# AHupuJR/REFID

Measured on AMD Instinct MI355X. Metric: interpolated frames/sec (train step) GoPro 256x256 11+1, higher is better.
Workload: dtype f32

## Files before the change

refid_amd/csrc/wgrad_wino24.hip:

```cpp
#include "common.h"
#include "wgrad_args.h"
#include <cstdlib>
#include <cstring>
#include <type_traits>
#include <vector>

#ifndef REFID_W24_ABLATE
#define REFID_W24_ABLATE 0
#endif
#define W24_NO_DMA (REFID_W24_ABLATE == 1 || REFID_W24_ABLATE == 5 || REFID_W24_ABLATE == 6)
#define W24_NO_MFMA (REFID_W24_ABLATE == 2)
#define W24_NO_LDS (REFID_W24_ABLATE == 3 || REFID_W24_ABLATE == 6)
#define W24_NO_BAR (REFID_W24_ABLATE == 4 || REFID_W24_ABLATE == 5 || REFID_W24_ABLATE == 6)

namespace {

__device__ __forceinline__ float w24_fake(float seed) { asm volatile("" : "+v"(seed)); return seed; }

constexpr int IT = 32;
constexpr int TC = 4;
constexpr int GH = 4, GW = 4 * TC;
constexpr int XH = GH + 2, XW = GW + 2;
constexpr int X_BYTES = XH * XW * IT * 4;
constexpr int GS_BYTES = GH * GW * 32 * 4;
constexpr int buf_bytes(int ns) { return X_BYTES + ns * GS_BYTES; }
constexpr int lds24_bytes(int ns) { return 2 * buf_bytes(ns); }
constexpr int NXI = 24;
typedef __attribute__((address_space(3))) void* lds_ptr24;
typedef __attribute__((address_space(3))) const float lds_cf24;
typedef float f32x2 __attribute__((ext_vector_type(2)));

template <int AH, int BH>
__device__ __forceinline__ f32x2 w24_pair(f32x2 a, f32x2 b) {
    f32x2 d;
    if constexpr (AH == 0 && BH == 0) asm("v_pk_mov_b32 %0, %1, %2 op_sel:[0,0]" : "=v"(d) : "v"(a), "v"(b));
    else if constexpr (AH == 1 && BH == 0) asm("v_pk_mov_b32 %0, %1, %2 op_sel:[1,0]" : "=v"(d) : "v"(a), "v"(b));
    else if constexpr (AH == 0 && BH == 1) asm("v_pk_mov_b32 %0, %1, %2 op_sel:[0,1]" : "=v"(d) : "v"(a), "v"(b));
    else asm("v_pk_mov_b32 %0, %1, %2 op_sel:[1,1]" : "=v"(d) : "v"(a), "v"(b));
    return d;
}

struct W24Args {
    const float* g[REFID_WGRAD_MAX_GROUPS]; const float* inA[REFID_WGRAD_MAX_GROUPS]; const float* inB[REFID_WGRAD_MAX_GROUPS];
    int groups;
    int ldG, Co;
    int ldA, ldB, Ca, Ctot;
    float* slabs; float* bslabs;
    int N, H, W, Ho, Wo, pad;
    int tilesX, tilesY, ntiles, nsplit;
    int CoP, CiP;
    int accum;
    int Hin, Win, ncoT;
};

template <int I>
struct W24Row {
    static constexpr int XR = XW * IT, GR = GW * 32, GSUB = GH * GW * 32;
    static constexpr int XA = I == 0 ? 0 : (I == 2 ? 2 : (I == 3 ? 3 : 1));
    static constexpr int XB = I == 0 ? 2 : (I == 2 ? 1 : (I == 3 ? 1 : 2));
    static constexpr bool XPLUS = I == 1;

    template <class T>
    static __device__ __forceinline__ T x_comb(T a, T b) { return XPLUS ? a + b : a - b; }
    static __device__ __forceinline__ void x_rows(lds_cf24* const (&xb)[4], int s, f32x2 (&t)[6]) {
#pragma unroll
        for (int c = 0; c < 4; ++c) {
            const int col = 4 * s + 2 + c;
            lds_cf24* p = xb[col & 3] + (col & ~3) * IT;
            const f32x2 a = W24_NO_LDS ? f32x2{w24_fake(1.f + c), w24_fake(2.f)} : f32x2{p[XA * XR], p[XA * XR + 4 * IT]};
            const f32x2 b = W24_NO_LDS ? f32x2{w24_fake(3.f + c), w24_fake(4.f)} : f32x2{p[XB * XR], p[XB * XR + 4 * IT]};
            t[2 + c] = x_comb(a, b);
        }
    }
    static __device__ __forceinline__ f32x2 x_rows01(lds_cf24* xe) {
        if (W24_NO_LDS) return f32x2{w24_fake(5.f), w24_fake(6.f)};
        return x_comb(f32x2{xe[XA * XR], xe[XA * XR + IT]}, f32x2{xe[XB * XR], xe[XB * XR + IT]});
    }
    static __device__ __forceinline__ void g_rows(lds_cf24* const (&gb)[4], int s, int sub, f32x2 (&x)[4]) {
#pragma unroll
        for (int c = 0; c < 4; ++c) {
            const int col = 4 * s + c;
            lds_cf24* p = gb[col & 3] + sub * GSUB + (col & ~3) * 32;
            if (W24_NO_LDS) { x[c] = f32x2{w24_fake(7.f + c), w24_fake(8.f + sub)}; continue; }
            if constexpr (I == 0) x[c] = f32x2{p[0], p[4 * 32]};
            else if constexpr (I == 3) x[c] = f32x2{p[GR], p[GR + 4 * 32]};
            else {
                const f32x2 g0 = f32x2{p[0], p[4 * 32]}, g1 = f32x2{p[GR], p[GR + 4 * 32]};
                x[c] = I == 1 ? g0 + g1 : g0 - g1;
            }
        }
    }
    static __device__ __forceinline__ void v_cols(const f32x2 (&t)[6], f32x2 (&v)[6]) {
        v[0] = 4.f * t[0] + (-5.f * t[2] + t[4]);
        v[1] = (t[3] + t[4]) - 4.f * (t[1] + t[2]);
        v[2] = 4.f * (t[1] - t[2]) + (t[4] - t[3]);
        const f32x2 d42 = t[4] - t[2], d31 = t[3] - t[1];
        v[3] = 2.f * d31 + d42;
        v[4] = d42 - 2.f * d31;
        v[5] = 4.f * t[1] + (-5.f * t[3] + t[5]);
    }
    static __device__ __forceinline__ void z_cols(const f32x2 (&x)[4], f32x2 (&z)[6]) {
        const f32x2 e = x[0] + x[2], o = x[1] + x[3], e4 = 4.f * x[2] + x[0], o4 = 4.f * x[3] + x[1];
        z[0] = x[0]; z[1] = e + o; z[2] = e - o; z[3] = 2.f * o4 + e4; z[4] = e4 - 2.f * o4; z[5] = x[3];
    }
};

template <int NS, bool DOWN>
__global__ __launch_bounds__(256, NS == 2 ? 2 : 3) void wgrad_wino24_kernel(const W24Args a) {
    constexpr int OT = 32 * NS, BUF_BYTES = buf_bytes(NS), XPS = DOWN ? 2 : 1;
    extern __shared__ __attribute__((aligned(16))) char smem[];
    const int tid = threadIdx.x, lane = tid & 63;
    const int wave = __builtin_amdgcn_readfirstlane(tid >> 6);
    const int li = lane & 31, kh = lane >> 5;
    const int phase = DOWN ? blockIdx.z / a.ncoT : 0, php = phase >> 1, phq = phase & 1;
    const int co0 = (DOWN ? blockIdx.z % a.ncoT : blockIdx.z) * OT, ci0 = blockIdx.y * IT;
    const int split = blockIdx.x;
    const int Hin = DOWN ? a.Hin : a.H, Win = DOWN ? a.Win : a.W;

    const bool xFromA = ci0 < a.Ca || ci0 >= a.Ctot;
    const int xld = xFromA ? a.ldA : a.ldB;
    const long long gpixAll = (long long)a.N * a.Ho * a.Wo, xpixAll = (long long)a.N * Hin * Win;
    const int limG = (int)min(gpixAll * a.ldG * 4, 0x7fffffffLL), limX = (int)min(xpixAll * xld * 4, 0x7fffffffLL);
    const int ntAll = a.ntiles * a.groups;
    const int chunk = (ntAll + a.nsplit - 1) / a.nsplit;
    const int p0 = min(split * chunk, ntAll), p1 = min(p0 + chunk, ntAll);

    int qg, qn, qy, qx;
    {
        int t = p0 < ntAll ? p0 : 0;
        qg = t / a.ntiles; t -= qg * a.ntiles;
        qx = t % a.tilesX; t /= a.tilesX;
        qy = t % a.tilesY; qn = t / a.tilesY;
    }
    const int xq = ci0 + (lane & 7) * 4, xt = ci0 + (lane & 31), gq = co0 + (lane & 7) * 4;
    const int xlc = ((lane >> 3) * XPS * xld + (xFromA ? xq : xq - a.Ca)) * 4;
    const int xlt = ((lane >> 5) * XPS * xld + (xFromA ? xt : xt - a.Ca)) * 4;
    const int glc = ((lane >> 3) * a.ldG + gq) * 4;
    const bool fullch = ci0 + IT <= a.Ctot && co0 + OT <= a.Co;
    constexpr int OOB = 0x7ff00000;
    const int xRowB = XPS * Win * xld * 4, gRowB = a.Wo * a.ldG * 4;
    auto x_origin = [&](int n, int ty, int tx) {
        return ((n * Hin + XPS * (ty * GH - a.pad) + php) * Win + XPS * (tx * GW - a.pad) + phq) * xld * 4;
    };
    const float* gPtr = a.g[qg];
    const float* xPtr = xFromA ? a.inA[qg] : a.inB[qg];
    int xTile = x_origin(qn, qy, qx);
    int gTile = ((qn * a.Ho + qy * GH) * a.Wo + qx * GW) * a.ldG * 4;
    auto request = [&](int buf) {
        const int oy0 = qy * GH, ox0 = qx * GW;
        const int iy0 = oy0 - a.pad, ix0 = ox0 - a.pad;
        const __amdgpu_buffer_rsrc_t rsG = __builtin_amdgcn_make_buffer_rsrc(const_cast<float*>(gPtr), 0, limG, 0x00020000);
        const __amdgpu_buffer_rsrc_t rsX = __builtin_amdgcn_make_buffer_rsrc(const_cast<float*>(xPtr), 0, limX, 0x00020000);
        char* xdst = smem + buf * BUF_BYTES;
        char* gdst = xdst + X_BYTES;
        const bool fast = fullch && ix0 >= 0 && ix0 + XW <= a.W && ox0 + GW <= a.Wo && xld * 8 * XPS * 4 < 0x100000 && a.ldG * 8 * 4 < 0x100000;
        const int q0 = NS == 2 ? (wave < 2 ? wave : 3 * wave - 4) : 2 * (wave - 2), nq = NS == 2 ? (wave < 2 ? 1 : 3) : (wave < 2 ? 0 : 2);
        if (fast) {
#pragma unroll
            for (int k = 0; k < 2; ++k) {
                const int r = wave + 4 * k;
                if (r < XH && !W24_NO_DMA) {
                    const int base = (unsigned)(iy0 + r) < (unsigned)a.H ? xTile + r * xRowB : OOB;
                    char* dst = xdst + r * (XW * IT * 4);
                    __builtin_amdgcn_raw_ptr_buffer_load_lds(rsX, (lds_ptr24)dst, 16, base + xlc, 0, 0, 0);
                    __builtin_amdgcn_raw_ptr_buffer_load_lds(rsX, (lds_ptr24)(dst + 1024), 16, base + 8 * XPS * xld * 4 + xlc, 0, 0, 0);
                    __builtin_amdgcn_raw_ptr_buffer_load_lds(rsX, (lds_ptr24)(dst + 2048), 4, base + 16 * XPS * xld * 4 + xlt, 0, 0, 0);
                }
            }
#pragma unroll
            for (int k = 0; k < 3; ++k) {
                if (k < nq && !W24_NO_DMA) {
                    const int q = q0 + k, r = q & 3, sub = q >> 2;
                    const int base = oy0 + r < a.Ho ? gTile + r * gRowB + sub * 128 : OOB;
                    char* dst = gdst + sub * GS_BYTES + r * (GW * 32 * 4);
                    __builtin_amdgcn_raw_ptr_buffer_load_lds(rsG, (lds_ptr24)dst, 16, base + glc, 0, 0, 0);
                    __builtin_amdgcn_raw_ptr_buffer_load_lds(rsG, (lds_ptr24)(dst + 1024), 16, base + 8 * a.ldG * 4 + glc, 0, 0, 0);
                }
            }
        } else {
            const int l8 = lane >> 3, l32 = lane >> 5;
            const int xbadq = xq < a.Ctot ? 0 : -1, xbadt = xt < a.Ctot ? 0 : -1;
            const int gbad0 = gq < a.Co ? 0 : -1, gbad1 = gq + 32 < a.Co ? 0 : -1;
            const int cx0 = (unsigned)(ix0 + l8) < (unsigned)a.W ? 0 : -1;
            const int cx1 = (unsigned)(ix0 + 8 + l8) < (unsigned)a.W ? 0 : -1;
            const int cxt = (unsigned)(ix0 + 16 + l32) < (unsigned)a.W ? 0 : -1;
            const int cg0 = ox0 + l8 < a.Wo ? 0 : -1, cg1 = ox0 + 8 + l8 < a.Wo ? 0 : -1;
#pragma unroll
            for (int k = 0; k < 2; ++k) {
                const int r = wave + 4 * k;
                if (r < XH && !W24_NO_DMA) {
                    const int rbad = (unsigned)(iy0 + r) < (unsigned)a.H ? 0 : -1;
                    const int base = xTile + r * xRowB;
                    char* dst = xdst + r * (XW * IT * 4);
                    __builtin_amdgcn_raw_ptr_buffer_load_lds(rsX, (lds_ptr24)dst, 16, (base + xlc) | xbadq | rbad | cx0, 0, 0, 0);
                    __builtin_amdgcn_raw_ptr_buffer_load_lds(rsX, (lds_ptr24)(dst + 1024), 16,
                                                             (base + 8 * XPS * xld * 4 + xlc) | xbadq | rbad | cx1, 0, 0, 0);
                    __builtin_amdgcn_raw_ptr_buffer_load_lds(rsX, (lds_ptr24)(dst + 2048), 4,
                                                             (base + 16 * XPS * xld * 4 + xlt) | xbadt | rbad | cxt, 0, 0, 0);
                }
            }
#pragma unroll
            for (int k = 0; k < 3; ++k) {
                if (k < nq && !W24_NO_DMA) {
                    const int q = q0 + k, r = q & 3, sub = q >> 2;
                    const int rbad = oy0 + r < a.Ho ? 0 : -1;
                    const int base = gTile + r * gRowB + sub * 128;
                    const int gbad = sub ? gbad1 : gbad0;
                    char* dst = gdst + sub * GS_BYTES + r * (GW * 32 * 4);
                    __builtin_amdgcn_raw_ptr_buffer_load_lds(rsG, (lds_ptr24)dst, 16, (base + glc) | gbad | rbad | cg0, 0, 0, 0);
                    __builtin_amdgcn_raw_ptr_buffer_load_lds(rsG, (lds_ptr24)(dst + 1024), 16,
                                                             (base + 8 * a.ldG * 4 + glc) | gbad | rbad | cg1, 0, 0, 0);
                }
            }
        }
        if (REFID_W24_ABLATE == 7) return;
        qx += 1;
        if (qx != a.tilesX) {
            xTile += GW * XPS * xld * 4;
            gTile += GW * a.ldG * 4;
        } else {
            qx = 0;
            qy += 1;
            if (qy == a.tilesY) {
                qy = 0;
                qn += 1;
                if (qn == a.N) {
                    qn = 0;
                    qg = min(qg + 1, a.groups - 1);
                    gPtr = a.g[qg];
                    xPtr = xFromA ? a.inA[qg] : a.inB[qg];
                }
            }
            xTile = x_origin(qn, qy, 0);
            gTile = (qn * a.Ho + qy * GH) * a.Wo * a.ldG * 4;
        }
    };

    f32x16 acc[6][NS];
#pragma unroll
    for (int j = 0; j < 6; ++j)
#pragma unroll
        for (int sm = 0; sm < NS; ++sm)
#pragma unroll
            for (int r = 0; r < 16; ++r) acc[j][sm][r] = 0.f;
    float bs[NS];
#pragma unroll
    for (int sm = 0; sm < NS; ++sm) bs[sm] = 0.f;

    static_assert(BUF_BYTES % 256 == 0 && (BUF_BYTES + X_BYTES + (NS - 1) * GS_BYTES + 4 * GW * 32 * 4) / 256 < 256, "ds_read2st64 offset range");
    lds_cf24* xe = (lds_cf24*)smem + (2 * kh) * (XW * IT) + li;
    lds_cf24* ge = (lds_cf24*)(smem + X_BYTES) + (2 * kh) * (GW * 32) + li;
    lds_cf24* xb[4] = {xe, xe + IT, xe + 2 * IT, xe + 3 * IT};
    lds_cf24* gb[4] = {ge, ge + 32, ge + 2 * 32, ge + 3 * 32};
    asm volatile("" : "+v"(xb[0]), "+v"(xb[1]), "+v"(xb[2]), "+v"(xb[3]), "+v"(xe));
    asm volatile("" : "+v"(gb[0]), "+v"(gb[1]), "+v"(gb[2]), "+v"(gb[3]));

    auto kloop = [&](auto TI) {
        constexpr int I = decltype(TI)::value;
        using R = W24Row<I>;
        auto tile = [&](auto BUF) {
            constexpr int BO = decltype(BUF)::value * (BUF_BYTES / 4);
            lds_cf24* xbb[4] = {xb[0] + BO, xb[1] + BO, xb[2] + BO, xb[3] + BO};
            lds_cf24* gbb[4] = {gb[0] + BO, gb[1] + BO, gb[2] + BO, gb[3] + BO};
            f32x2 t[6], p4, p5;
#pragma unroll
            for (int s = 0; s < TC; s += 2) {
                R::x_rows(xbb, s, t);
                if (s == 0) {
                    const f32x2 a01 = R::x_rows01(xe + BO);
                    t[0] = w24_pair<0, 0>(a01, t[4]);
                    t[1] = w24_pair<1, 0>(a01, t[5]);
                } else {
                    t[0] = w24_pair<1, 0>(p4, t[4]);
                    t[1] = w24_pair<1, 0>(p5, t[5]);
                }
                p4 = t[4]; p5 = t[5];
                f32x2 v[6];
                R::v_cols(t, v);
#pragma unroll
                for (int sm = 0; sm < NS; ++sm) {
                    f32x2 x[4], z[6];
                    R::g_rows(gbb, s, sm, x);
                    R::z_cols(x, z);
                    if constexpr (I == 1) bs[sm] += z[1][0] + z[1][1];
#pragma unroll
                    for (int h = 0; h < 2; ++h)
#pragma unroll
                        for (int j = 0; j < 6; ++j) {
                            if (W24_NO_MFMA) { asm volatile("" :: "v"(v[j][h]), "v"(z[j][h])); continue; }
                            acc[j][sm] = __builtin_amdgcn_mfma_f32_32x32x2f32(v[j][h], z[j][h], acc[j][sm], 0, 0, 0);
                        }
                }
            }
        };
        auto sync = [&] {
            __builtin_amdgcn_s_waitcnt(0x0F70);
            if (!W24_NO_BAR) __builtin_amdgcn_s_barrier();
            __builtin_amdgcn_sched_barrier(0);
        };
        const int npairs = (p1 - p0) >> 1;
        if (p0 < p1) request(0);
        for (int i = 0; i < npairs; ++i) {
            sync();
            request(1);
            tile(std::integral_constant<int, 0>{});
            sync();
            if (p0 + 2 * i + 2 < p1) request(0);
            tile(std::integral_constant<int, 1>{});
        }
        if ((p1 - p0) & 1) {
            sync();
            tile(std::integral_constant<int, 0>{});
        }
    };
    switch (wave) {
        case 0: kloop(std::integral_constant<int, 0>{}); break;
        case 1: kloop(std::integral_constant<int, 1>{}); break;
        case 2: kloop(std::integral_constant<int, 2>{}); break;
        default: kloop(std::integral_constant<int, 3>{}); break;
    }

#pragma unroll
    for (int j = 0; j < 6; ++j) {
        float* sl = a.slabs + ((long long)((split * (DOWN ? 4 : 1) + phase) * NXI + wave * 6 + j) * a.CoP) * a.CiP;
#pragma unroll
        for (int sm = 0; sm < NS; ++sm) {
            const int co = co0 + sm * 32 + li;
#pragma unroll
            for (int qd = 0; qd < 4; ++qd) {
                const int ci = ci0 + 8 * qd + 4 * kh;
                f32x4 vv;
#pragma unroll
                for (int k = 0; k < 4; ++k) vv[k] = acc[j][sm][4 * qd + k];
                f32x4* dst = reinterpret_cast<f32x4*>(sl + (long long)co * a.CiP + ci);
                if (a.accum) vv += *dst;
                *dst = vv;
            }
        }
    }
    if (a.bslabs != nullptr && blockIdx.y == 0 && phase == 0 && wave == 1) {
#pragma unroll
        for (int sm = 0; sm < NS; ++sm) {
            const float tot = bs[sm] + __shfl_xor(bs[sm], 32, 64);
            if (kh == 0) {
                float* dst = a.bslabs + (long long)split * a.CoP + co0 + sm * 32 + li;
                *dst = a.accum ? *dst + tot : tot;
            }
        }
    }
}

struct W24rArgs {
    const float* slabs; const float* bslabs; float* dw; float* db;
    int nsplit, Co, Ci, CoP, CiP, iBase, iTotal, perGroup;
    int nsplitW;
    int down;
};

__device__ __forceinline__ void w24_fold_body(const float* __restrict__ slabs, float* __restrict__ part, long long slabFloats,
                                              int nsplit, int S, int piece, int s) {
    const long long off = ((long long)piece * 256 + threadIdx.x) * 4;
    if (off >= slabFloats) return;
    const f32x4* p = reinterpret_cast<const f32x4*>(slabs + off);
    const long long st4 = slabFloats / 4;
    f32x4 a0 = {0.f, 0.f, 0.f, 0.f}, a1 = a0;
    int k = s;
    for (; k + S < nsplit; k += 2 * S) { a0 += p[k * st4]; a1 += p[(k + S) * st4]; }
    if (k < nsplit) a0 += p[k * st4];
    *reinterpret_cast<f32x4*>(part + (long long)s * slabFloats + off) = a0 + a1;
}
__global__ __launch_bounds__(256) void wgrad_wino24_fold_kernel(const float* __restrict__ slabs, float* __restrict__ part,
                                                                long long slabFloats, int nsplit, int S) {
    w24_fold_body(slabs, part, slabFloats, nsplit, S, blockIdx.x, blockIdx.y);
}

constexpr int FOLD_BATCH = 96;
struct FoldJob { const float* slabs; float* part; long long slabFloats; int nsplit, S; };
struct FoldBatch { FoldJob job[FOLD_BATCH]; int blk0[FOLD_BATCH + 1]; int n; };
static_assert(sizeof(FoldBatch) <= 4096, "kernel-argument block");
__global__ __launch_bounds__(256) void wgrad_fold_batch_kernel(const FoldBatch b) {
    int j = 0;
    for (int k = 1; k < b.n; ++k) j = (int)blockIdx.x >= b.blk0[k] ? k : j;
    const FoldJob& f = b.job[j];
    const int blk = (int)blockIdx.x - b.blk0[j];
    const int pieces = (int)((f.slabFloats / 4 + 255) / 256);
    w24_fold_body(f.slabs, f.part, f.slabFloats, f.nsplit, f.S, blk % pieces, blk / pieces);
}
thread_local std::vector<FoldJob> fold_queue;

__device__ __forceinline__ void w24_reduce_body(const W24rArgs& a, const int blk, float* part) {
    const long long plane = (long long)a.CoP * a.CiP;
    const long long slabStride = NXI * plane;
    const int lpe = a.perGroup, eb = 256 / lpe;
    const int el = threadIdx.x % eb, sub = threadIdx.x / eb;
    const long long e = (long long)blk * eb + el;
    const bool live = e < (long long)a.Co * a.Ci;
    const int ci = live ? (int)(e % a.Ci) : 0, co = live ? (int)(e / a.Ci) : 0;
    {
        const float* p = a.slabs + (long long)co * a.CiP + ci;
        float u[NXI];
#pragma unroll
        for (int x = 0; x < NXI; ++x) u[x] = 0.f;
        if (live) {
            for (int k = sub; k < a.nsplitW; k += lpe) {
#pragma unroll
                for (int x = 0; x < NXI; ++x) u[x] += p[k * slabStride + x * plane];
            }
        }
        if (lpe > 1) {
#pragma unroll
            for (int x = 0; x < NXI; ++x) part[threadIdx.x * (NXI + 1) + x] = u[x];
            __syncthreads();
            if (sub == 0) {
                for (int s2 = 1; s2 < lpe; ++s2) {
#pragma unroll
                    for (int x = 0; x < NXI; ++x) u[x] += part[(s2 * eb + el) * (NXI + 1) + x];
                }
            }
        }
        if (live && sub == 0) {
            constexpr float c4 = 0.25f, c6 = 1.f / 6.f, c12 = 1.f / 12.f, c24 = 1.f / 24.f;
            float dg[9];
#pragma unroll
            for (int pp = 0; pp < 3; ++pp) {
                float t[6];
#pragma unroll
                for (int j = 0; j < 6; ++j) {
                    const float m = 0.5f * (u[6 + j] + u[12 + j]), d = 0.5f * (u[6 + j] - u[12 + j]);
                    t[j] = pp == 0 ? u[j] + m : (pp == 1 ? d : m + u[18 + j]);
                }
                const float s12 = t[1] + t[2], d21 = t[2] - t[1], s34 = t[3] + t[4], d34 = t[3] - t[4];
                dg[pp * 3 + 0] = c4 * t[0] - c6 * s12 + c24 * s34;
                dg[pp * 3 + 1] = c6 * d21 + c12 * d34;
                dg[pp * 3 + 2] = c6 * (s34 - s12) + t[5];
            }
            float* dst = a.dw + ((long long)co * a.iTotal + a.iBase + ci) * 9;
#pragma unroll
            for (int k = 0; k < 9; ++k) dst[k] += dg[k];
        }
    }
    if (a.db != nullptr && blk == 0) {
        for (int c2 = threadIdx.x; c2 < a.Co; c2 += 256) {
            float s = 0.f;
            for (int k = 0; k < a.nsplit; ++k) s += a.bslabs[(long long)k * a.CoP + c2];
            a.db[c2] += s;
        }
    }
}

__global__ __launch_bounds__(256) void wgrad_wino24_reduce_kernel(const W24rArgs a) {
    __shared__ float part[256 * (NXI + 1)];
    w24_reduce_body(a, blockIdx.x, part);
}

__device__ __forceinline__ void w24_reduce_down_body(const W24rArgs& a, const int blk) {
    const long long plane = (long long)a.CoP * a.CiP;
    const long long slabStride = 4 * NXI * plane;
    const long long gid = (long long)blk * 256 + threadIdx.x;
    const long long e = gid >> 2;
    const int ph = (int)(gid & 3);
    const bool live = e < (long long)a.Co * a.Ci;
    const int ci = live ? (int)(e % a.Ci) : 0, co = live ? (int)(e / a.Ci) : 0;
    if (live) {
        const float* p = a.slabs + (long long)co * a.CiP + ci + ph * NXI * plane;
        float u[NXI];
#pragma unroll
        for (int x = 0; x < NXI; ++x) u[x] = 0.f;
        for (int k = 0; k < a.nsplitW; ++k) {
#pragma unroll
            for (int x = 0; x < NXI; ++x) u[x] += p[k * slabStride + x * plane];
        }
        constexpr float c4 = 0.25f, c6 = 1.f / 6.f, c12 = 1.f / 12.f, c24 = 1.f / 24.f;
        float* dst = a.dw + ((long long)co * a.iTotal + a.iBase + ci) * 16;
#pragma unroll
        for (int pp = 0; pp < 3; ++pp) {
            const int ky = 2 * pp + (ph >> 1) - 1;
            float t[6];
#pragma unroll
            for (int j = 0; j < 6; ++j) {
                const float m = 0.5f * (u[6 + j] + u[12 + j]), d = 0.5f * (u[6 + j] - u[12 + j]);
                t[j] = pp == 0 ? u[j] + m : (pp == 1 ? d : m + u[18 + j]);
            }
            const float s12 = t[1] + t[2], d21 = t[2] - t[1], s34 = t[3] + t[4], d34 = t[3] - t[4];
            const float r3[3] = {c4 * t[0] - c6 * s12 + c24 * s34, c6 * d21 + c12 * d34, c6 * (s34 - s12) + t[5]};
            if (ky < 0 || ky > 3) continue;
#pragma unroll
            for (int q = 0; q < 3; ++q) {
                const int kx = 2 * q + (ph & 1) - 1;
                if (kx >= 0 && kx <= 3) dst[ky * 4 + kx] += r3[q];
            }
        }
    }
    if (a.db != nullptr && blk == 0) {
        for (int c2 = threadIdx.x; c2 < a.Co; c2 += 256) {
            float sacc = 0.f;
            for (int k = 0; k < a.nsplit; ++k) sacc += a.bslabs[(long long)k * a.CoP + c2];
            a.db[c2] += sacc;
        }
    }
}

__global__ __launch_bounds__(256) void wgrad_wino24_reduce_down_kernel(const W24rArgs a) { w24_reduce_down_body(a, blockIdx.x); }

struct W24rBatch { W24rArgs job[REFID_FINISH_BATCH]; int blk0[REFID_FINISH_BATCH + 1]; int n; };
static_assert(sizeof(W24rBatch) <= 4096, "kernel-argument block");
__global__ __launch_bounds__(256) void wgrad_wino24_reduce_batch_kernel(const W24rBatch b) {
    __shared__ float part[256 * (NXI + 1)];
    int j = 0;
    for (int k = 1; k < b.n; ++k) j = (int)blockIdx.x >= b.blk0[k] ? k : j;
    const int blk = (int)blockIdx.x - b.blk0[j];
    if (b.job[j].down) w24_reduce_down_body(b.job[j], blk);
    else w24_reduce_body(b.job[j], blk, part);
}

struct W24rQueued { W24rArgs r; int nblocks; };
thread_local std::vector<W24rQueued> w24_queue;

struct Geo24 { int ncoT, nciT, tilesX, tilesY, ntiles, nsplit, CoP, CiP; };

int ns_of(const refid_wgrad_desc* d) { return d->c_o <= 32 ? 1 : 2; }
bool is_down(const refid_wgrad_desc* d) { return d->kh == 4; }

Geo24 geo24_of(const refid_wgrad_desc* d) {
    Geo24 g;
    const int OT = 32 * ns_of(d);
    g.ncoT = cdiv(d->c_o, OT);
    const int ci_geo = (d->phase != 0) ? d->i_total - d->i_base : d->c_a + d->c_b;
    g.nciT = cdiv(ci_geo > d->c_a + d->c_b ? ci_geo : d->c_a + d->c_b, IT);
    g.tilesX = cdiv(d->wo, GW);
    g.tilesY = cdiv(d->ho, GH);
    g.ntiles = g.tilesX * g.tilesY * d->n;
    static const int wgs = []() { const char* e = getenv("REFID_W24_WGS"); return e ? atoi(e) : 512; }();
    int want = cdiv(ns_of(d) == 1 ? wgs * 3 / 2 : wgs, g.ncoT * g.nciT * (is_down(d) ? 4 : 1));
    if (want >= 8) want = want / 8 * 8;
    if (want < 1) want = 1;
    if (want > g.ntiles) want = g.ntiles;
    g.nsplit = want;
    g.CoP = g.ncoT * OT;
    g.CiP = g.nciT * IT;
    return g;
}

}

int refid_slab_fold_count(long long slabFloats, int nsplit) {
    if (nsplit < 2) return 0;
    const long long pieces = (slabFloats / 4 + 255) / 256;
    int S = (int)((2048 + pieces - 1) / pieces);
    if (S > 16) S = 16;
    if (S >= nsplit) S = nsplit / 2;
    return S < 1 ? 1 : S;
}
int refid_launch_slab_fold(const float* slabs, float* part, long long slabFloats, int nsplit, int S, hipStream_t st) {
    static const bool batch_folds = !(getenv("REFID_FOLD_BATCH") && getenv("REFID_FOLD_BATCH")[0] == '0');
    if (batch_folds && refid_finish_defer_now()) {
        fold_queue.push_back({slabs, part, slabFloats, nsplit, S});
        return 0;
    }
    hipLaunchKernelGGL(wgrad_wino24_fold_kernel, dim3((unsigned)((slabFloats / 4 + 255) / 256), S), dim3(256), 0, st, slabs, part,
                       slabFloats, nsplit, S);
    REFID_LAUNCH_CHECK("wgrad_slab_fold");
    return 0;
}

int refid_slab_fold_flush(hipStream_t st) {
    size_t at = 0;
    while (at < fold_queue.size()) {
        FoldBatch b;
        memset(&b, 0, sizeof(b));
        int n = 0;
        long long blk = 0;
        for (; n < FOLD_BATCH && at < fold_queue.size(); ++n, ++at) {
            const FoldJob& f = fold_queue[at];
            const long long nb = ((f.slabFloats / 4 + 255) / 256) * f.S;
            if (n > 0 && blk + nb > 0x3fffffffLL) break;
            b.job[n] = f;
            b.blk0[n] = (int)blk;
            blk += nb;
        }
        b.blk0[n] = (int)blk; b.n = n;
        hipLaunchKernelGGL(wgrad_fold_batch_kernel, dim3((unsigned)blk), dim3(256), 0, st, b);
        if (hipGetLastError() != hipSuccess) { fold_queue.clear(); refid_set_error("wgrad_fold_batch: launch failed"); return 1; }
    }
    fold_queue.clear();
    return 0;
}

int refid_wino24_finish_flush(hipStream_t st) {
    size_t at = 0;
    while (at < w24_queue.size()) {
        W24rBatch b;
        memset(&b, 0, sizeof(b));
        int n = 0, blk = 0;
        for (; n < REFID_FINISH_BATCH && at < w24_queue.size(); ++n, ++at) {
            b.job[n] = w24_queue[at].r;
            b.blk0[n] = blk;
            blk += w24_queue[at].nblocks;
        }
        b.blk0[n] = blk; b.n = n;
        hipLaunchKernelGGL(wgrad_wino24_reduce_batch_kernel, dim3(blk), dim3(256), 0, st, b);
        if (hipGetLastError() != hipSuccess) { w24_queue.clear(); refid_set_error("wgrad_wino24_reduce_batch: launch failed"); return 1; }
    }
    w24_queue.clear();
    return 0;
}

namespace {
long long slab_floats(const refid_wgrad_desc* d, const Geo24& g) { return (long long)(is_down(d) ? 4 : 1) * NXI * g.CoP * g.CiP; }
}

size_t refid_wgrad_wino24_workspace_bytes(const refid_wgrad_desc* d) {
    const Geo24 g = geo24_of(d);
    const long long slab = slab_floats(d, g);
    return ((size_t)g.nsplit * slab + (size_t)g.nsplit * g.CoP + (size_t)refid_slab_fold_count(slab, g.nsplit) * slab) * sizeof(float);
}

int refid_wgrad_wino24_launch(const refid_wgrad_desc* d, hipStream_t st) {
    static std::atomic<unsigned long long> attr_done{0}, attr_done1{0}, attr_done2{0}, attr_done3{0};
    if (int rc = refid_lds_attr_once(attr_done, &wgrad_wino24_kernel<2, false>, lds24_bytes(2), "wgrad_wino24")) return rc;
    if (int rc = refid_lds_attr_once(attr_done1, &wgrad_wino24_kernel<1, false>, lds24_bytes(1), "wgrad_wino24<1>")) return rc;
    if (int rc = refid_lds_attr_once(attr_done2, &wgrad_wino24_kernel<2, true>, lds24_bytes(2), "wgrad_wino24<down>")) return rc;
    if (int rc = refid_lds_attr_once(attr_done3, &wgrad_wino24_kernel<1, true>, lds24_bytes(1), "wgrad_wino24<1, down>")) return rc;
    const Geo24 g = geo24_of(d);
    const bool down = is_down(d);
    const long long slab = slab_floats(d, g);
    if (down)
        REFID_CHECK(d->kw == 4 && d->stride == 2 && d->pad == 1 && d->h % 2 == 0 && d->w % 2 == 0 && d->ho == d->h / 2 && d->wo == d->w / 2,
                    "wgrad (algo 7): a 4x4 stride-2 pad-1 conv over an even-sized input");
    REFID_CHECK(d->c_b == 0 || d->c_a % IT == 0, "wgrad (Winograd 2x4 tiles): c_a must be a multiple of %d for two sources", IT);
    REFID_CHECK(d->ld_g % 4 == 0 && d->ld_a % 4 == 0 && (d->c_b == 0 || d->ld_b % 4 == 0) && d->c_o % 4 == 0 &&
                    d->c_a % 4 == 0 && d->c_b % 4 == 0,
                "wgrad (Winograd 2x4 tiles): pitches and channel counts must be multiples of 4 floats (16-byte LDS-DMA pieces)");
    {
        const long long lim = 0x7fffffffLL;
        REFID_CHECK((long long)d->n * d->ho * d->wo * d->ld_g * 4 < lim && (long long)d->n * d->h * d->w * d->ld_a * 4 < lim &&
                        (d->c_b == 0 || (long long)d->n * d->h * d->w * d->ld_b * 4 < lim),
                    "wgrad (Winograd 2x4 tiles): tensor too large for 32-bit buffer offsets (use algo 0)");
    }
    W24Args a;
    const int ngrp = d->groups > 1 ? d->groups : 1;
    REFID_CHECK(ngrp <= REFID_WGRAD_MAX_GROUPS, "wgrad: at most %d grouped time steps", REFID_WGRAD_MAX_GROUPS);
    for (int k = 0; k < REFID_WGRAD_MAX_GROUPS; ++k) {
        const bool on = k > 0 && k < ngrp;
        a.g[k] = k == 0 ? d->g : (on ? d->g_more[k - 1] : d->g);
        a.inA[k] = k == 0 ? d->in_a : (on ? d->in_a_more[k - 1] : d->in_a);
        a.inB[k] = k == 0 ? d->in_b : (on ? d->in_b_more[k - 1] : d->in_b);
        REFID_CHECK(a.g[k] && a.inA[k] && (d->c_b == 0 || a.inB[k]), "wgrad: null tensor pointer in group %d", k);
        REFID_CHECK(((uintptr_t)a.g[k] | (uintptr_t)a.inA[k] | (uintptr_t)(d->c_b ? a.inB[k] : nullptr)) % 16 == 0,
                    "wgrad (Winograd 2x4 tiles): tensors must be 16-byte aligned (group %d)", k);
    }
    a.groups = ngrp;
    a.ldG = d->ld_g; a.Co = d->c_o;
    a.ldA = d->ld_a; a.ldB = d->ld_b;
    a.Ca = d->c_a; a.Ctot = d->c_a + d->c_b;
    a.slabs = d->slabs;
    a.bslabs = d->db ? d->slabs + (size_t)g.nsplit * slab : nullptr;
    a.N = d->n; a.H = d->h; a.W = d->w; a.Ho = d->ho; a.Wo = d->wo; a.pad = d->pad;
    a.Hin = d->h; a.Win = d->w; a.ncoT = g.ncoT;
    if (down) { a.H = d->ho; a.W = d->wo; a.pad = 1; }
    a.tilesX = g.tilesX; a.tilesY = g.tilesY; a.ntiles = g.ntiles; a.nsplit = g.nsplit;
    a.CoP = g.CoP; a.CiP = g.CiP;
    a.accum = (d->phase == 2);
    if (d->phase != 3) {
        if (down) {
            if (ns_of(d) == 1)
                hipLaunchKernelGGL((wgrad_wino24_kernel<1, true>), dim3(g.nsplit, g.nciT, 4 * g.ncoT), dim3(256), lds24_bytes(1), st, a);
            else
                hipLaunchKernelGGL((wgrad_wino24_kernel<2, true>), dim3(g.nsplit, g.nciT, 4 * g.ncoT), dim3(256), lds24_bytes(2), st, a);
        } else if (ns_of(d) == 1)
            hipLaunchKernelGGL((wgrad_wino24_kernel<1, false>), dim3(g.nsplit, g.nciT, g.ncoT), dim3(256), lds24_bytes(1), st, a);
        else
            hipLaunchKernelGGL((wgrad_wino24_kernel<2, false>), dim3(g.nsplit, g.nciT, g.ncoT), dim3(256), lds24_bytes(2), st, a);
        REFID_LAUNCH_CHECK("wgrad_wino24");
    }
    if (d->phase == 1 || d->phase == 2) return 0;
    W24rArgs r;
    r.slabs = a.slabs; r.bslabs = a.bslabs; r.dw = d->dw; r.db = d->db;
    r.nsplit = g.nsplit; r.Co = d->o_real;
    int nred = g.nsplit;
    if (const int S = refid_slab_fold_count(slab, g.nsplit)) {
        const long long slabFloats = slab;
        float* part = d->slabs + (size_t)g.nsplit * slab + (size_t)g.nsplit * g.CoP;
        if (int rc = refid_launch_slab_fold(a.slabs, part, slabFloats, g.nsplit, S, st)) return rc;
        r.slabs = part;
        nred = S;
    }
    r.Ci = (d->phase == 0 && a.Ctot < d->i_total - d->i_base) ? a.Ctot : d->i_total - d->i_base;
    r.CoP = g.CoP; r.CiP = g.CiP; r.iBase = d->i_base; r.iTotal = d->i_total;
    const long long total = (long long)r.Co * r.Ci;
    int lpe = 1;
    while (lpe < 16 && (long long)lpe * 2 * total <= 65536 && lpe * 2 <= nred) lpe *= 2;
    r.perGroup = lpe;
    r.nsplitW = nred;
    r.down = down ? 1 : 0;
    if (refid_finish_defer_now()) {
        for (const W24rQueued& q : w24_queue)
            if (q.r.dw == r.dw && q.r.iBase == r.iBase) {
                if (int rc = refid_slab_fold_flush(st)) return rc;
                if (int rc = refid_wino24_finish_flush(st)) return rc;
                break;
            }
        w24_queue.push_back({r, down ? (int)((total * 4 + 255) / 256) : (int)((total + 256 / lpe - 1) / (256 / lpe))});
        return 0;
    }
    if (down) {
        hipLaunchKernelGGL(wgrad_wino24_reduce_down_kernel, dim3((int)((total * 4 + 255) / 256)), dim3(256), 0, st, r);
        REFID_LAUNCH_CHECK("wgrad_wino24_reduce_down");
        return 0;
    }
    hipLaunchKernelGGL(wgrad_wino24_reduce_kernel, dim3((int)((total + 256 / lpe - 1) / (256 / lpe))), dim3(256), 0, st, r);
    REFID_LAUNCH_CHECK("wgrad_wino24_reduce");
    return 0;
}
```

Measured before the change: 525.6.

## Add eight-wave Winograd wgrad variant sharing gradient tiles across two input-channel blocks

Adds an X8 form of the Winograd 2x4 weight-gradient kernel with 512 threads. Two groups of four waves each handle a 32-channel input block and share one staged gradient tile in LDS. The new form uses a triple-buffered LDS pipeline with partial waitcnt so two tile loads can be in flight. It is meant to halve gradient tile traffic per input channel and to hide load latency better. In exchange it runs at one workgroup per CU with a larger LDS footprint. It is selected by default for non-down 64-output-channel layers with at least 256x256 output pixels and more than 32 input channels.

Measured after the change: 529.5 (median of 6 runs). Within noise of the previous version (+0.7%).

```diff
diff --git a/refid_amd/csrc/wgrad_wino24.hip b/refid_amd/csrc/wgrad_wino24.hip
--- a/refid_amd/csrc/wgrad_wino24.hip
+++ b/refid_amd/csrc/wgrad_wino24.hip
@@ -16,6 +16,11 @@
 namespace {
 
 __device__ __forceinline__ float w24_fake(float seed) { asm volatile("" : "+v"(seed)); return seed; }
+__device__ __forceinline__ int w24_lane_now() {
+    int l;
+    asm volatile("v_mbcnt_lo_u32_b32 %0, -1, 0\n\tv_mbcnt_hi_u32_b32 %0, -1, %0" : "=v"(l));
+    return l;
+}
 
 constexpr int IT = 32;
 constexpr int TC = 4;
@@ -25,6 +30,9 @@
 constexpr int GS_BYTES = GH * GW * 32 * 4;
 constexpr int buf_bytes(int ns) { return X_BYTES + ns * GS_BYTES; }
 constexpr int lds24_bytes(int ns) { return 2 * buf_bytes(ns); }
+constexpr int X8_XOFF(int h, int b) { return (3 * h + b) * X_BYTES; }
+constexpr int X8_GOFF(int b) { return 6 * X_BYTES + b * 2 * GS_BYTES; }
+constexpr int LDS24X8_BYTES = X8_GOFF(3);
 constexpr int NXI = 24;
 typedef __attribute__((address_space(3))) void* lds_ptr24;
 typedef __attribute__((address_space(3))) const float lds_cf24;
@@ -105,15 +113,17 @@
     }
 };
 
-template <int NS, bool DOWN>
-__global__ __launch_bounds__(256, NS == 2 ? 2 : 3) void wgrad_wino24_kernel(const W24Args a) {
+template <int NS, bool DOWN, bool X8 = false>
+__global__ __launch_bounds__(X8 ? 512 : 256, X8 ? 1 : (NS == 2 ? 2 : 3)) void wgrad_wino24_kernel(const W24Args a) {
+    static_assert(!X8 || (NS == 2 && !DOWN), "the eight-wave form is the 64-output-channel 3x3 tile");
     constexpr int OT = 32 * NS, BUF_BYTES = buf_bytes(NS), XPS = DOWN ? 2 : 1;
     extern __shared__ __attribute__((aligned(16))) char smem[];
     const int tid = threadIdx.x, lane = tid & 63;
     const int wave = __builtin_amdgcn_readfirstlane(tid >> 6);
+    const int row = wave & 3, hx = X8 ? wave >> 2 : 0;
     const int li = lane & 31, kh = lane >> 5;
     const int phase = DOWN ? blockIdx.z / a.ncoT : 0, php = phase >> 1, phq = phase & 1;
-    const int co0 = (DOWN ? blockIdx.z % a.ncoT : blockIdx.z) * OT, ci0 = blockIdx.y * IT;
+    const int co0 = (DOWN ? blockIdx.z % a.ncoT : blockIdx.z) * OT, ci0 = (X8 ? 2 : 1) * blockIdx.y * IT + hx * IT;
     const int split = blockIdx.x;
     const int Hin = DOWN ? a.Hin : a.H, Win = DOWN ? a.Win : a.W;
 
@@ -151,14 +161,15 @@
         const int iy0 = oy0 - a.pad, ix0 = ox0 - a.pad;
         const __amdgpu_buffer_rsrc_t rsG = __builtin_amdgcn_make_buffer_rsrc(const_cast<float*>(gPtr), 0, limG, 0x00020000);
         const __amdgpu_buffer_rsrc_t rsX = __builtin_amdgcn_make_buffer_rsrc(const_cast<float*>(xPtr), 0, limX, 0x00020000);
-        char* xdst = smem + buf * BUF_BYTES;
-        char* gdst = xdst + X_BYTES;
+        char* xdst = smem + (X8 ? X8_XOFF(hx, buf) : buf * BUF_BYTES);
+        char* gdst = X8 ? smem + X8_GOFF(buf) : xdst + X_BYTES;
         const bool fast = fullch && ix0 >= 0 && ix0 + XW <= a.W && ox0 + GW <= a.Wo && xld * 8 * XPS * 4 < 0x100000 && a.ldG * 8 * 4 < 0x100000;
-        const int q0 = NS == 2 ? (wave < 2 ? wave : 3 * wave - 4) : 2 * (wave - 2), nq = NS == 2 ? (wave < 2 ? 1 : 3) : (wave < 2 ? 0 : 2);
+        const int q0 = X8 ? wave : (NS == 2 ? (wave < 2 ? wave : 3 * wave - 4) : 2 * (wave - 2));
+        const int nq = X8 ? 1 : (NS == 2 ? (wave < 2 ? 1 : 3) : (wave < 2 ? 0 : 2));
         if (fast) {
 #pragma unroll
             for (int k = 0; k < 2; ++k) {
-                const int r = wave + 4 * k;
+                const int r = row + 4 * k;
                 if (r < XH && !W24_NO_DMA) {
                     const int base = (unsigned)(iy0 + r) < (unsigned)a.H ? xTile + r * xRowB : OOB;
                     char* dst = xdst + r * (XW * IT * 4);
@@ -187,7 +198,7 @@
             const int cg0 = ox0 + l8 < a.Wo ? 0 : -1, cg1 = ox0 + 8 + l8 < a.Wo ? 0 : -1;
 #pragma unroll
             for (int k = 0; k < 2; ++k) {
-                const int r = wave + 4 * k;
+                const int r = row + 4 * k;
                 if (r < XH && !W24_NO_DMA) {
                     const int rbad = (unsigned)(iy0 + r) < (unsigned)a.H ? 0 : -1;
                     const int base = xTile + r * xRowB;
@@ -247,9 +258,13 @@
 #pragma unroll
     for (int sm = 0; sm < NS; ++sm) bs[sm] = 0.f;
 
+    constexpr int NBUF = X8 ? 3 : 2;
+    constexpr int XSTEP = X8 ? X_BYTES : BUF_BYTES, GSTEP = X8 ? 2 * GS_BYTES : BUF_BYTES;
     static_assert(BUF_BYTES % 256 == 0 && (BUF_BYTES + X_BYTES + (NS - 1) * GS_BYTES + 4 * GW * 32 * 4) / 256 < 256, "ds_read2st64 offset range");
-    lds_cf24* xe = (lds_cf24*)smem + (2 * kh) * (XW * IT) + li;
-    lds_cf24* ge = (lds_cf24*)(smem + X_BYTES) + (2 * kh) * (GW * 32) + li;
+    static_assert(X_BYTES % 256 == 0 && (2 * X_BYTES + X_BYTES) / 256 < 256 && (2 * 2 * GS_BYTES + 2 * GS_BYTES) / 256 < 256,
+                  "ds_read2st64 offset range (X8)");
+    lds_cf24* xe = (lds_cf24*)(smem + (X8 ? X8_XOFF(hx, 0) : 0)) + (2 * kh) * (XW * IT) + li;
+    lds_cf24* ge = (lds_cf24*)(smem + (X8 ? X8_GOFF(0) : X_BYTES)) + (2 * kh) * (GW * 32) + li;
     lds_cf24* xb[4] = {xe, xe + IT, xe + 2 * IT, xe + 3 * IT};
     lds_cf24* gb[4] = {ge, ge + 32, ge + 2 * 32, ge + 3 * 32};
     asm volatile("" : "+v"(xb[0]), "+v"(xb[1]), "+v"(xb[2]), "+v"(xb[3]), "+v"(xe));
@@ -259,9 +274,9 @@
         constexpr int I = decltype(TI)::value;
         using R = W24Row<I>;
         auto tile = [&](auto BUF) {
-            constexpr int BO = decltype(BUF)::value * (BUF_BYTES / 4);
+            constexpr int BO = decltype(BUF)::value * (XSTEP / 4), GO = decltype(BUF)::value * (GSTEP / 4);
             lds_cf24* xbb[4] = {xb[0] + BO, xb[1] + BO, xb[2] + BO, xb[3] + BO};
-            lds_cf24* gbb[4] = {gb[0] + BO, gb[1] + BO, gb[2] + BO, gb[3] + BO};
+            lds_cf24* gbb[4] = {gb[0] + GO, gb[1] + GO, gb[2] + GO, gb[3] + GO};
             f32x2 t[6], p4, p5;
 #pragma unroll
             for (int s = 0; s < TC; s += 2) {
@@ -298,37 +313,72 @@
             if (!W24_NO_BAR) __builtin_amdgcn_s_barrier();
             __builtin_amdgcn_sched_barrier(0);
         };
-        const int npairs = (p1 - p0) >> 1;
-        if (p0 < p1) request(0);
-        for (int i = 0; i < npairs; ++i) {
-            sync();
-            request(1);
-            tile(std::integral_constant<int, 0>{});
-            sync();
-            if (p0 + 2 * i + 2 < p1) request(0);
-            tile(std::integral_constant<int, 1>{});
-        }
-        if ((p1 - p0) & 1) {
-            sync();
-            tile(std::integral_constant<int, 0>{});
+        constexpr int NV = (I < 2 ? 2 : 1) * 3 + 2;
+        auto sync_lead = [&](bool next_in_flight) {
+            if (next_in_flight) __builtin_amdgcn_s_waitcnt(0x0F70 | NV);
+            else __builtin_amdgcn_s_waitcnt(0x0F70);
+            if (!W24_NO_BAR) __builtin_amdgcn_s_barrier();
+            __builtin_amdgcn_sched_barrier(0);
+        };
+        const int n = p1 - p0;
+        if constexpr (NBUF == 3) {
+            const int ntriples = n / 3;
+            if (n > 0) request(0);
+            if (n > 1) request(1);
+            for (int i = 0; i < ntriples; ++i) {
+                const int t = 3 * i;
+                sync_lead(t + 1 < n);
+                if (t + 2 < n) request(2);
+                tile(std::integral_constant<int, 0>{});
+                sync_lead(t + 2 < n);
+                if (t + 3 < n) request(0);
+                tile(std::integral_constant<int, 1>{});
+                sync_lead(t + 3 < n);
+                if (t + 4 < n) request(1);
+                tile(std::integral_constant<int, 2>{});
+            }
+            if (n % 3 != 0) {
+                sync_lead(n % 3 == 2);
+                tile(std::integral_constant<int, 0>{});
+            }
+            if (n % 3 == 2) {
+                sync_lead(false);
+                tile(std::integral_constant<int, 1>{});
+            }
+        } else {
+            const int npairs = n >> 1;
+            if (p0 < p1) request(0);
+            for (int i = 0; i < npairs; ++i) {
+                sync();
+                request(1);
+                tile(std::integral_constant<int, 0>{});
+                sync();
+                if (p0 + 2 * i + 2 < p1) request(0);
+                tile(std::integral_constant<int, 1>{});
+            }
+            if (n & 1) {
+                sync();
+                tile(std::integral_constant<int, 0>{});
+            }
         }
     };
-    switch (wave) {
+    switch (row) {
         case 0: kloop(std::integral_constant<int, 0>{}); break;
         case 1: kloop(std::integral_constant<int, 1>{}); break;
         case 2: kloop(std::integral_constant<int, 2>{}); break;
         default: kloop(std::integral_constant<int, 3>{}); break;
     }
 
+    const int lane_e = X8 ? w24_lane_now() : lane, li_e = lane_e & 31, kh_e = lane_e >> 5;
 #pragma unroll
     for (int j = 0; j < 6; ++j) {
-        float* sl = a.slabs + ((long long)((split * (DOWN ? 4 : 1) + phase) * NXI + wave * 6 + j) * a.CoP) * a.CiP;
+        float* sl = a.slabs + ((long long)((split * (DOWN ? 4 : 1) + phase) * NXI + row * 6 + j) * a.CoP) * a.CiP;
 #pragma unroll
         for (int sm = 0; sm < NS; ++sm) {
-            const int co = co0 + sm * 32 + li;
+            const int co = co0 + sm * 32 + li_e;
 #pragma unroll
             for (int qd = 0; qd < 4; ++qd) {
-                const int ci = ci0 + 8 * qd + 4 * kh;
+                const int ci = ci0 + 8 * qd + 4 * kh_e;
                 f32x4 vv;
 #pragma unroll
                 for (int k = 0; k < 4; ++k) vv[k] = acc[j][sm][4 * qd + k];
@@ -342,8 +392,8 @@
 #pragma unroll
         for (int sm = 0; sm < NS; ++sm) {
             const float tot = bs[sm] + __shfl_xor(bs[sm], 32, 64);
-            if (kh == 0) {
-                float* dst = a.bslabs + (long long)split * a.CoP + co0 + sm * 32 + li;
+            if (kh_e == 0) {
+                float* dst = a.bslabs + (long long)split * a.CoP + co0 + sm * 32 + li_e;
                 *dst = a.accum ? *dst + tot : tot;
             }
         }
@@ -516,28 +566,40 @@
 struct W24rQueued { W24rArgs r; int nblocks; };
 thread_local std::vector<W24rQueued> w24_queue;
 
-struct Geo24 { int ncoT, nciT, tilesX, tilesY, ntiles, nsplit, CoP, CiP; };
+struct Geo24 { int ncoT, nciT, tilesX, tilesY, ntiles, nsplit, CoP, CiP; bool x8; };
 
 int ns_of(const refid_wgrad_desc* d) { return d->c_o <= 32 ? 1 : 2; }
 bool is_down(const refid_wgrad_desc* d) { return d->kh == 4; }
+
+constexpr long long X8_MIN_PIXELS = 256 * 256;
+bool use_x8(const refid_wgrad_desc* d, int ci_geo) {
+    const char* e = getenv("REFID_WGRAD_W24X8");
+    const int mode = e && e[0] ? atoi(e) : -1;
+    if (mode == 0 || is_down(d) || ns_of(d) != 2 || ci_geo <= IT) return false;
+    return mode == 1 || (long long)d->ho * d->wo >= X8_MIN_PIXELS;
+}
 
 Geo24 geo24_of(const refid_wgrad_desc* d) {
     Geo24 g;
     const int OT = 32 * ns_of(d);
     g.ncoT = cdiv(d->c_o, OT);
     const int ci_geo = (d->phase != 0) ? d->i_total - d->i_base : d->c_a + d->c_b;
-    g.nciT = cdiv(ci_geo > d->c_a + d->c_b ? ci_geo : d->c_a + d->c_b, IT);
+    const int ci_t = ci_geo > d->c_a + d->c_b ? ci_geo : d->c_a + d->c_b;
+    g.x8 = use_x8(d, ci_t);
+    const int ITW = g.x8 ? 2 * IT : IT;
+    g.nciT = cdiv(ci_t, ITW);
     g.tilesX = cdiv(d->wo, GW);
     g.tilesY = cdiv(d->ho, GH);
     g.ntiles = g.tilesX * g.tilesY * d->n;
     static const int wgs = []() { const char* e = getenv("REFID_W24_WGS"); return e ? atoi(e) : 512; }();
-    int want = cdiv(ns_of(d) == 1 ? wgs * 3 / 2 : wgs, g.ncoT * g.nciT * (is_down(d) ? 4 : 1));
+    static const int wgs8 = []() { const char* e = getenv("REFID_W24X8_WGS"); return e ? atoi(e) : 256; }();
+    int want = cdiv(g.x8 ? wgs8 : (ns_of(d) == 1 ? wgs * 3 / 2 : wgs), g.ncoT * g.nciT * (is_down(d) ? 4 : 1));
     if (want >= 8) want = want / 8 * 8;
     if (want < 1) want = 1;
     if (want > g.ntiles) want = g.ntiles;
     g.nsplit = want;
     g.CoP = g.ncoT * OT;
-    g.CiP = g.nciT * IT;
+    g.CiP = g.nciT * ITW;
     return g;
 }
 
@@ -616,11 +678,12 @@
 }
 
 int refid_wgrad_wino24_launch(const refid_wgrad_desc* d, hipStream_t st) {
-    static std::atomic<unsigned long long> attr_done{0}, attr_done1{0}, attr_done2{0}, attr_done3{0};
+    static std::atomic<unsigned long long> attr_done{0}, attr_done1{0}, attr_done2{0}, attr_done3{0}, attr_done8{0};
     if (int rc = refid_lds_attr_once(attr_done, &wgrad_wino24_kernel<2, false>, lds24_bytes(2), "wgrad_wino24")) return rc;
     if (int rc = refid_lds_attr_once(attr_done1, &wgrad_wino24_kernel<1, false>, lds24_bytes(1), "wgrad_wino24<1>")) return rc;
     if (int rc = refid_lds_attr_once(attr_done2, &wgrad_wino24_kernel<2, true>, lds24_bytes(2), "wgrad_wino24<down>")) return rc;
     if (int rc = refid_lds_attr_once(attr_done3, &wgrad_wino24_kernel<1, true>, lds24_bytes(1), "wgrad_wino24<1, down>")) return rc;
+    if (int rc = refid_lds_attr_once(attr_done8, &wgrad_wino24_kernel<2, false, true>, LDS24X8_BYTES, "wgrad_wino24<x8>")) return rc;
     const Geo24 g = geo24_of(d);
     const bool down = is_down(d);
     const long long slab = slab_floats(d, g);
@@ -667,7 +730,9 @@
                 hipLaunchKernelGGL((wgrad_wino24_kernel<1, true>), dim3(g.nsplit, g.nciT, 4 * g.ncoT), dim3(256), lds24_bytes(1), st, a);
             else
                 hipLaunchKernelGGL((wgrad_wino24_kernel<2, true>), dim3(g.nsplit, g.nciT, 4 * g.ncoT), dim3(256), lds24_bytes(2), st, a);
-        } else if (ns_of(d) == 1)
+        } else if (g.x8)
+            hipLaunchKernelGGL((wgrad_wino24_kernel<2, false, true>), dim3(g.nsplit, g.nciT, g.ncoT), dim3(512), LDS24X8_BYTES, st, a);
+        else if (ns_of(d) == 1)
             hipLaunchKernelGGL((wgrad_wino24_kernel<1, false>), dim3(g.nsplit, g.nciT, g.ncoT), dim3(256), lds24_bytes(1), st, a);
         else
             hipLaunchKernelGGL((wgrad_wino24_kernel<2, false>), dim3(g.nsplit, g.nciT, g.ncoT), dim3(256), lds24_bytes(2), st, a);
```
